# CVPR23/Depth-guided-Texture-Diffusion-for-Image-Semantic-Segmentation

Hardware: NVIDIA B200
Metric: rgbd_images_per_sec_384 (higher is better)
Workload: dtype bf16

## Files before the change

### depth-guided-texture-diffusion-for-image-semantic-segmentation_b200/csrc/common.cuh

```cuda
#pragma once
#include <cuda_bf16.h>
#include <cuda_runtime.h>
#include <stdint.h>
#include <stdio.h>

#include "../../include/dgtd_ops.h"

#if defined(__CUDA_ARCH__) && (__CUDA_ARCH__ < 1000)
#error "libdgtd_ops targets sm_100a only"
#endif

namespace dgtd {

void set_error(const char* fmt, ...);
void count_launch(int n = 1);

#define DGTD_CHECK_ARG(cond, ...)        \
  do {                                   \
    if (!(cond)) {                       \
      ::dgtd::set_error(__VA_ARGS__);    \
      return -1;                         \
    }                                    \
  } while (0)

#define DGTD_LAUNCH_CHECK(name)                                                  \
  do {                                                                           \
    cudaError_t e__ = cudaGetLastError();                                        \
    if (e__ != cudaSuccess) {                                                    \
      ::dgtd::set_error("%s: launch failed: %s", name, cudaGetErrorString(e__)); \
      return -2;                                                                 \
    }                                                                            \
    ::dgtd::count_launch();                                                      \
  } while (0)

static inline int cdiv(int64_t a, int64_t b) { return (int)((a + b - 1) / b); }

__device__ __forceinline__ float warp_sum(float v) {
#pragma unroll
  for (int o = 16; o > 0; o >>= 1) v += __shfl_xor_sync(0xffffffffu, v, o);
  return v;
}

__device__ __forceinline__ float gelu_erf(float x) {
  return 0.5f * x * (1.0f + erff(x * 0.70710678118654752440f));
}

__device__ __forceinline__ float sigmoidf_acc(float x) { return 1.0f / (1.0f + expf(-x)); }

template <int ACT>
__device__ __forceinline__ float apply_act(float x) {
  if (ACT == DGTD_ACT_GELU) return gelu_erf(x);
  if (ACT == DGTD_ACT_RELU) return fmaxf(x, 0.0f);
  return x;
}

__device__ __forceinline__ float to_float(float v) { return v; }
__device__ __forceinline__ float to_float(__nv_bfloat16 v) { return __bfloat162float(v); }

template <typename T>
__device__ __forceinline__ T from_float(float v);
template <>
__device__ __forceinline__ float from_float<float>(float v) { return v; }
template <>
__device__ __forceinline__ __nv_bfloat16 from_float<__nv_bfloat16>(float v) {
  return __float2bfloat16_rn(v);
}

__device__ __forceinline__ void store1(float* p, float v) { *p = v; }
__device__ __forceinline__ void store1(__nv_bfloat16* p, float v) { *p = __float2bfloat16_rn(v); }
__device__ __forceinline__ void store4(float* p, float a, float b, float c, float d) {
  *reinterpret_cast<float4*>(p) = make_float4(a, b, c, d);
}
__device__ __forceinline__ void store4(__nv_bfloat16* p, float a, float b, float c, float d) {
  __nv_bfloat162 lo = __floats2bfloat162_rn(a, b), hi = __floats2bfloat162_rn(c, d);
  uint2 u;
  u.x = *reinterpret_cast<uint32_t*>(&lo);
  u.y = *reinterpret_cast<uint32_t*>(&hi);
  *reinterpret_cast<uint2*>(p) = u;
}
__device__ __forceinline__ float4 load4(const float* p) {
  return *reinterpret_cast<const float4*>(p);
}
__device__ __forceinline__ float4 load4(const __nv_bfloat16* p) {
  uint2 u = *reinterpret_cast<const uint2*>(p);
  __nv_bfloat162 lo = *reinterpret_cast<__nv_bfloat162*>(&u.x);
  __nv_bfloat162 hi = *reinterpret_cast<__nv_bfloat162*>(&u.y);
  float2 a = __bfloat1622float2(lo), b = __bfloat1622float2(hi);
  return make_float4(a.x, a.y, b.x, b.y);
}

__device__ __forceinline__ uint64_t pk2(float a, float b) {
  uint64_t r;
  asm("mov.b64 %0, {%1, %2};" : "=l"(r) : "f"(a), "f"(b));
  return r;
}
__device__ __forceinline__ void up2(uint64_t r, float& a, float& b) {
  asm("mov.b64 {%0, %1}, %2;" : "=f"(a), "=f"(b) : "l"(r));
}
__device__ __forceinline__ uint64_t fma2(uint64_t a, uint64_t b, uint64_t c) {
  uint64_t d;
  asm("fma.rn.f32x2 %0, %1, %2, %3;" : "=l"(d) : "l"(a), "l"(b), "l"(c));
  return d;
}
__device__ __forceinline__ uint64_t mul2(uint64_t a, uint64_t b) {
  uint64_t d;
  asm("mul.rn.f32x2 %0, %1, %2;" : "=l"(d) : "l"(a), "l"(b));
  return d;
}
__device__ __forceinline__ uint64_t add2(uint64_t a, uint64_t b) {
  uint64_t d;
  asm("add.rn.f32x2 %0, %1, %2;" : "=l"(d) : "l"(a), "l"(b));
  return d;
}
__device__ __forceinline__ void bilinear_src(int dst, float scale, int in_size, int& i0, int& i1,
                                             float& l1) {
  float s = (dst + 0.5f) * scale - 0.5f;
  s = s < 0.f ? 0.f : s;
  i0 = (int)s;
  if (i0 > in_size - 1) i0 = in_size - 1;
  i1 = i0 + (i0 < in_size - 1 ? 1 : 0);
  l1 = s - (float)i0;
}

}
```

### depth-guided-texture-diffusion-for-image-semantic-segmentation_b200/csrc/dwconv_tma.cu

```cuda
#include "blackwell.cuh"
#include "common.cuh"

namespace dgtd {

int sm_count();
static inline int sm_count_dw() { return sm_count(); }

template <int SY, int SX, bool ADD, typename OT = float>
__global__ void __launch_bounds__(SY * SX * 32, 2)
dwconv7_tma_kernel(const __grid_constant__ CUtensorMap tmX, const float* __restrict__ wT,
                   const float* __restrict__ bias, const float* __restrict__ add, OT* __restrict__ y, int h,
                   int w, int C, int tiles_x, int tiles_y) {
  constexpr int TH = 4 * SY, TW = 8 * SX, PH = TH + 6, PW = TW + 6, NCH = 4;
  constexpr int TILE_FLOATS = PH * PW * 32;
  constexpr uint32_t TILE_BYTES = TILE_FLOATS * 4;
  extern __shared__ __align__(128) float xs[];
  __shared__ uint64_t bar[2];

  int bid = blockIdx.x;
  const int cgs = C >> 7;
  const int cg = bid % cgs; bid /= cgs;
  const int tx = bid % tiles_x; bid /= tiles_x;
  const int ty = bid % tiles_y;
  const int b = bid / tiles_y;
  const int warp = threadIdx.x >> 5, lane = threadIdx.x & 31;
  const int sy = warp / SX, sx = warp - sy * SX;
  const int x0 = tx * TW, y0 = ty * TH;

  if (threadIdx.x == 0) {
    bw::prefetch_tmap(&tmX);
    bw::mbar_init(&bar[0], 1);
    bw::mbar_init(&bar[1], 1);
    bw::fence_mbar_init();
  }
  __syncthreads();
  if (threadIdx.x == 0) {
    bw::mbar_arrive_expect_tx(&bar[0], TILE_BYTES);
    bw::tma_load_4d(&tmX, &bar[0], xs, cg * 128, x0 - 3, y0 - 3, b);
  }

#pragma unroll 1
  for (int i = 0; i < NCH; ++i) {
    const int c = cg * 128 + i * 32 + lane;
    if (threadIdx.x == 0 && i + 1 < NCH) {
      bw::fence_proxy_async_smem();
      bw::mbar_arrive_expect_tx(&bar[(i + 1) & 1], TILE_BYTES);
      bw::tma_load_4d(&tmX, &bar[(i + 1) & 1], xs + ((i + 1) & 1) * TILE_FLOATS, cg * 128 + (i + 1) * 32, x0 - 3,
                      y0 - 3, b);
    }
    uint64_t w2[49];
#pragma unroll
    for (int k = 0; k < 49; ++k) {
      const float t = __ldg(wT + (int64_t)k * C + c);
      w2[k] = pk2(t, t);
    }
    const float bc = bias ? __ldg(bias + c) : 0.f;
    uint64_t acc[2][8];
#pragma unroll
    for (int q = 0; q < 2; ++q)
#pragma unroll
      for (int j = 0; j < 8; ++j) acc[q][j] = pk2(bc, bc);

    bw::mbar_wait(&bar[i & 1], (i >> 1) & 1);
    const float* base = xs + (i & 1) * TILE_FLOATS + ((4 * sy) * PW + 8 * sx) * 32 + lane;
#pragma unroll
    for (int iy = 0; iy < 9; ++iy) {
      uint64_t pr[14];
#pragma unroll
      for (int j = 0; j < 14; ++j) {
        const volatile float* p0 = base + (iy * PW + j) * 32;
        pr[j] = pk2(p0[0], p0[PW * 32]);
      }
#pragma unroll
      for (int q = 0; q < 2; ++q) {
        const int ky = iy - 2 * q;
        if (ky < 0 || ky >= 7) continue;
#pragma unroll
        for (int kx = 0; kx < 7; ++kx)
#pragma unroll
          for (int j = 0; j < 8; ++j) acc[q][j] = fma2(w2[ky * 7 + kx], pr[j + kx], acc[q][j]);
      }
    }
    if (ADD) {
      float av[4][8];
#pragma unroll
      for (int a = 0; a < 4; ++a)
#pragma unroll
        for (int j = 0; j < 8; ++j) {
          const int oy = y0 + 4 * sy + a, ox = x0 + 8 * sx + j;
          av[a][j] = (oy < h && ox < w) ? __ldg(add + (((int64_t)b * h + oy) * w + ox) * C + c) : 0.f;
        }
#pragma unroll
      for (int q = 0; q < 2; ++q)
#pragma unroll
        for (int j = 0; j < 8; ++j) acc[q][j] = add2(acc[q][j], pk2(av[2 * q][j], av[2 * q + 1][j]));
    }
    {
      const int oy0 = y0 + 4 * sy, ox0 = x0 + 8 * sx;
      OT* yp = y + (((int64_t)b * h + oy0) * w + ox0) * C + c;
      const int rs = w * C;
      if (oy0 + 4 <= h && ox0 + 8 <= w) {
#pragma unroll
        for (int q = 0; q < 2; ++q)
#pragma unroll
          for (int j = 0; j < 8; ++j) {
            float v0, v1;
            up2(acc[q][j], v0, v1);
            store1(yp + (2 * q) * rs + j * C, v0);
            store1(yp + (2 * q + 1) * rs + j * C, v1);
          }
      } else {
#pragma unroll
        for (int q = 0; q < 2; ++q)
#pragma unroll
          for (int j = 0; j < 8; ++j) {
            float v0, v1;
            up2(acc[q][j], v0, v1);
            if (ox0 + j < w) {
              if (oy0 + 2 * q < h) store1(yp + (2 * q) * rs + j * C, v0);
              if (oy0 + 2 * q + 1 < h) store1(yp + (2 * q + 1) * rs + j * C, v1);
            }
          }
      }
    }
    __syncthreads();
  }
}


template <int SY, int SX, bool ADD, typename OT>
__global__ void __launch_bounds__(SY * SX * 32, 2)
dwconv7_tma_persist_kernel(const __grid_constant__ CUtensorMap tmX, const __grid_constant__ CUtensorMap tmW,
                           const float* __restrict__ bias, const float* __restrict__ add, OT* __restrict__ y, int h,
                           int w, int C, int tiles_x, int tiles_y, int num_items) {
  constexpr int TH = 4 * SY, TW = 8 * SX, PH = TH + 6, PW = TW + 6;
  constexpr int TILE_FLOATS = PH * PW * 32;
  constexpr uint32_t TILE_BYTES = TILE_FLOATS * 4, W_BYTES = 49 * 32 * 4;
  extern __shared__ __align__(128) float xs[];
  float* wbuf = xs + 2 * TILE_FLOATS;
  __shared__ uint64_t bar[3];

  const int warp = threadIdx.x >> 5, lane = threadIdx.x & 31;
  const int sy = warp / SX, sx = warp - sy * SX;
  const int nch = C >> 5;
  auto issue_tile = [&](int item, int buf) {
    const int chunk = item % nch;
    int t = item / nch;
    const int tx = t % tiles_x; t /= tiles_x;
    const int ty = t % tiles_y;
    const int b = t / tiles_y;
    bw::mbar_arrive_expect_tx(&bar[buf], TILE_BYTES);
    bw::tma_load_4d(&tmX, &bar[buf], xs + buf * TILE_FLOATS, chunk * 32, tx * TW - 3, ty * TH - 3, b);
  };
  auto issue_weights = [&](int item) {
    bw::mbar_arrive_expect_tx(&bar[2], W_BYTES);
    bw::tma_load_2d(&tmW, &bar[2], wbuf, (item % nch) * 32, 0);
  };
  if (threadIdx.x == 0) {
    bw::prefetch_tmap(&tmX);
    bw::prefetch_tmap(&tmW);
    bw::mbar_init(&bar[0], 1);
    bw::mbar_init(&bar[1], 1);
    bw::mbar_init(&bar[2], 1);
    bw::fence_mbar_init();
  }
  __syncthreads();
  if (threadIdx.x == 0 && (int)blockIdx.x < num_items) {
    issue_tile(blockIdx.x, 0);
    issue_weights(blockIdx.x);
  }
  int it = 0;
#pragma unroll 1
  for (int item = blockIdx.x; item < num_items; item += gridDim.x, ++it) {
    const int next = item + gridDim.x;
    if (threadIdx.x == 0 && next < num_items) {
      bw::fence_proxy_async_smem();
      issue_tile(next, (it + 1) & 1);
    }
    const int chunk = item % nch;
    int t = item / nch;
    const int tx = t % tiles_x; t /= tiles_x;
    const int ty = t % tiles_y;
    const int b = t / tiles_y;
    const int x0 = tx * TW, y0 = ty * TH;
    const int c = chunk * 32 + lane;
    bw::mbar_wait(&bar[2], it & 1);
    uint64_t w2[49];
#pragma unroll
    for (int k = 0; k < 49; ++k) {
      const float tv = wbuf[k * 32 + lane];
      w2[k] = pk2(tv, tv);
    }
    __syncthreads();
    if (threadIdx.x == 0 && next < num_items) {
      bw::fence_proxy_async_smem();
      issue_weights(next);
    }
    const float bc = bias ? __ldg(bias + c) : 0.f;
    uint64_t acc[2][8];
#pragma unroll
    for (int q = 0; q < 2; ++q)
#pragma unroll
      for (int j = 0; j < 8; ++j) acc[q][j] = pk2(bc, bc);

    bw::mbar_wait(&bar[it & 1], (it >> 1) & 1);
    const float* base = xs + (it & 1) * TILE_FLOATS + ((4 * sy) * PW + 8 * sx) * 32 + lane;
#pragma unroll
    for (int iy = 0; iy < 9; ++iy) {
      uint64_t pr[14];
#pragma unroll
      for (int j = 0; j < 14; ++j) {
        const volatile float* p0 = base + (iy * PW + j) * 32;
        pr[j] = pk2(p0[0], p0[PW * 32]);
      }
#pragma unroll
      for (int q = 0; q < 2; ++q) {
        const int ky = iy - 2 * q;
        if (ky < 0 || ky >= 7) continue;
#pragma unroll
        for (int kx = 0; kx < 7; ++kx)
#pragma unroll
          for (int j = 0; j < 8; ++j) acc[q][j] = fma2(w2[ky * 7 + kx], pr[j + kx], acc[q][j]);
      }
    }
    if (ADD) {
      float av[4][8];
#pragma unroll
      for (int a = 0; a < 4; ++a)
#pragma unroll
        for (int j = 0; j < 8; ++j) {
          const int oy = y0 + 4 * sy + a, ox = x0 + 8 * sx + j;
          av[a][j] = (oy < h && ox < w) ? __ldg(add + (((int64_t)b * h + oy) * w + ox) * C + c) : 0.f;
        }
#pragma unroll
      for (int q = 0; q < 2; ++q)
#pragma unroll
        for (int j = 0; j < 8; ++j) acc[q][j] = add2(acc[q][j], pk2(av[2 * q][j], av[2 * q + 1][j]));
    }
    {
      const int oy0 = y0 + 4 * sy, ox0 = x0 + 8 * sx;
      OT* yp = y + (((int64_t)b * h + oy0) * w + ox0) * C + c;
      const int rs = w * C;
      if (oy0 + 4 <= h && ox0 + 8 <= w) {
#pragma unroll
        for (int q = 0; q < 2; ++q)
#pragma unroll
          for (int j = 0; j < 8; ++j) {
            float v0, v1;
            up2(acc[q][j], v0, v1);
            store1(yp + (2 * q) * rs + j * C, v0);
            store1(yp + (2 * q + 1) * rs + j * C, v1);
          }
      } else {
#pragma unroll
        for (int q = 0; q < 2; ++q)
#pragma unroll
          for (int j = 0; j < 8; ++j) {
            float v0, v1;
            up2(acc[q][j], v0, v1);
            if (ox0 + j < w) {
              if (oy0 + 2 * q < h) store1(yp + (2 * q) * rs + j * C, v0);
              if (oy0 + 2 * q + 1 < h) store1(yp + (2 * q + 1) * rs + j * C, v1);
            }
          }
      }
    }
    __syncthreads();
  }
}

template <int SY, int SX>
__global__ void __launch_bounds__(SY * SX * 32, 2)
dwconv7_wgrad_tma_kernel(const __grid_constant__ CUtensorMap tmX, const float* __restrict__ dy,
                         float* __restrict__ part, int h, int w, int C, int tiles_x, int tiles_y, int ntiles) {
  constexpr int TH = 4 * SY, TW = 8 * SX, PH = TH + 6, PW = TW + 6, NW = SY * SX;
  constexpr int TILE_FLOATS = PH * PW * 32;
  constexpr uint32_t TILE_BYTES = TILE_FLOATS * 4;
  static_assert(NW * 50 * 32 <= 2 * TILE_FLOATS, "reduction scratch must fit in the tile buffers");
  extern __shared__ __align__(128) float xs[];
  __shared__ uint64_t bar[2];

  const int chunk = blockIdx.x, P = gridDim.y;
  const int warp = threadIdx.x >> 5, lane = threadIdx.x & 31;
  const int sy = warp / SX, sx = warp - sy * SX;
  const int c = chunk * 32 + lane;

  auto issue = [&](int t, int buf) {
    const int tx = t % tiles_x;
    const int r = t / tiles_x;
    const int ty = r % tiles_y, b = r / tiles_y;
    bw::mbar_arrive_expect_tx(&bar[buf], TILE_BYTES);
    bw::tma_load_4d(&tmX, &bar[buf], xs + buf * TILE_FLOATS, chunk * 32, tx * TW - 3, ty * TH - 3, b);
  };
  if (threadIdx.x == 0) {
    bw::prefetch_tmap(&tmX);
    bw::mbar_init(&bar[0], 1);
    bw::mbar_init(&bar[1], 1);
    bw::fence_mbar_init();
  }
  __syncthreads();
  if (threadIdx.x == 0) issue(blockIdx.y, 0);

  float acc[50];
#pragma unroll
  for (int k = 0; k < 50; ++k) acc[k] = 0.f;

  int it = 0;
#pragma unroll 1
  for (int t = blockIdx.y; t < ntiles; t += P, ++it) {
    if (threadIdx.x == 0 && t + P < ntiles) {
      bw::fence_proxy_async_smem();
      issue(t + P, (it + 1) & 1);
    }
    const int tx = t % tiles_x;
    const int r = t / tiles_x;
    const int ty = r % tiles_y, b = r / tiles_y;
    const int oy0 = ty * TH + 4 * sy, ox0 = tx * TW + 8 * sx;
    float g[4][8];
#pragma unroll
    for (int a = 0; a < 4; ++a)
#pragma unroll
      for (int j = 0; j < 8; ++j) {
        const int oy = oy0 + a, ox = ox0 + j;
        g[a][j] = (oy < h && ox < w) ? __ldg(dy + (((int64_t)b * h + oy) * w + ox) * C + c) : 0.f;
        acc[49] += g[a][j];
      }
    bw::mbar_wait(&bar[it & 1], (it >> 1) & 1);
    const float* base = xs + (it & 1) * TILE_FLOATS + ((4 * sy) * PW + 8 * sx) * 32 + lane;
#pragma unroll
    for (int iy = 0; iy < 10; ++iy) {
      float in[14];
#pragma unroll
      for (int j = 0; j < 14; ++j) in[j] = base[(iy * PW + j) * 32];
#pragma unroll
      for (int a = 0; a < 4; ++a) {
        const int ky = iy - a;
        if (ky < 0 || ky >= 7) continue;
#pragma unroll
        for (int kx = 0; kx < 7; ++kx)
#pragma unroll
          for (int j = 0; j < 8; ++j) acc[ky * 7 + kx] = fmaf(g[a][j], in[j + kx], acc[ky * 7 + kx]);
      }
    }
    __syncthreads();
  }
  float* red = xs;
#pragma unroll
  for (int k = 0; k < 50; ++k) red[(warp * 50 + k) * 32 + lane] = acc[k];
  __syncthreads();
  for (int i = threadIdx.x; i < 50 * 32; i += NW * 32) {
    float v = 0.f;
#pragma unroll
    for (int q = 0; q < NW; ++q) v += red[q * 50 * 32 + i];
    part[((int64_t)blockIdx.y * 50 + (i >> 5)) * C + chunk * 32 + (i & 31)] = v;
  }
}

template <typename OT, int VPL>
__global__ void __launch_bounds__(256)
ln_rows_kernel(const float* __restrict__ y, const float* __restrict__ ln_w, const float* __restrict__ ln_b,
               OT* __restrict__ out, int64_t rows, int C, float eps) {
  const int64_t row = (int64_t)blockIdx.x * 8 + (threadIdx.x >> 5);
  if (row >= rows) return;
  const int lane = threadIdx.x & 31;
  const float* p = y + row * C;
  float4 v[VPL];
  float s = 0.f;
#pragma unroll
  for (int j = 0; j < VPL; ++j) {
    v[j] = *reinterpret_cast<const float4*>(p + (j * 32 + lane) * 4);
    s += (v[j].x + v[j].y) + (v[j].z + v[j].w);
  }
  const float mean = warp_sum(s) / C;
  float q = 0.f;
#pragma unroll
  for (int j = 0; j < VPL; ++j) {
    float a = v[j].x - mean, b = v[j].y - mean, c = v[j].z - mean, d = v[j].w - mean;
    q += (a * a + b * b) + (c * c + d * d);
  }
  const float rstd = 1.0f / sqrtf(warp_sum(q) / C + eps);
  OT* o = out + row * C;
#pragma unroll
  for (int j = 0; j < VPL; ++j) {
    const int c0 = (j * 32 + lane) * 4;
    float4 g = *reinterpret_cast<const float4*>(ln_w + c0), be = *reinterpret_cast<const float4*>(ln_b + c0);
    store4(o + c0, (v[j].x - mean) * rstd * g.x + be.x, (v[j].y - mean) * rstd * g.y + be.y,
           (v[j].z - mean) * rstd * g.z + be.z, (v[j].w - mean) * rstd * g.w + be.w);
  }
}

template <int LPR, int V, int U>
__global__ void __launch_bounds__(256)
row_stats_bf16_kernel(const __nv_bfloat16* __restrict__ y, float2* __restrict__ stats, int64_t rows, int C, float eps) {
  constexpr int RPP = 32 / LPR;
  constexpr int RPW = RPP * U;
  const int lane = threadIdx.x & 31, sub = lane / LPR, l = lane % LPR;
  const int64_t row0 = ((int64_t)blockIdx.x * 8 + (threadIdx.x >> 5)) * RPW + sub;
  uint4 raw[U][V];
#pragma unroll
  for (int u = 0; u < U; ++u) {
    const int64_t row = row0 + u * RPP;
#pragma unroll
    for (int j = 0; j < V; ++j) {
      raw[u][j] = make_uint4(0u, 0u, 0u, 0u);
      if (row < rows) raw[u][j] = __ldg(reinterpret_cast<const uint4*>(y + row * C + (j * LPR + l) * 8));
    }
  }
  const float inv_c = 1.0f / C;
#pragma unroll
  for (int u = 0; u < U; ++u) {
    float f[V][8];
    float s = 0.f;
#pragma unroll
    for (int j = 0; j < V; ++j) {
      const uint32_t w4[4] = {raw[u][j].x, raw[u][j].y, raw[u][j].z, raw[u][j].w};
#pragma unroll
      for (int e = 0; e < 4; ++e) {
        f[j][2 * e] = __uint_as_float(w4[e] << 16);
        f[j][2 * e + 1] = __uint_as_float(w4[e] & 0xffff0000u);
      }
      s += ((f[j][0] + f[j][1]) + (f[j][2] + f[j][3])) + ((f[j][4] + f[j][5]) + (f[j][6] + f[j][7]));
    }
#pragma unroll
    for (int o = LPR / 2; o > 0; o >>= 1) s += __shfl_xor_sync(0xffffffffu, s, o);
    const float mean = s * inv_c;
    float q = 0.f;
#pragma unroll
    for (int j = 0; j < V; ++j) {
#pragma unroll
      for (int e = 0; e < 8; e += 2) {
        const float a = f[j][e] - mean, b = f[j][e + 1] - mean;
        q += a * a + b * b;
      }
    }
#pragma unroll
    for (int o = LPR / 2; o > 0; o >>= 1) q += __shfl_xor_sync(0xffffffffu, q, o);
    const int64_t row = row0 + u * RPP;
    if (l == 0 && row < rows) stats[row] = make_float2(mean, 1.0f / sqrtf(q * inv_c + eps));
  }
}

static int row_stats_grid(int64_t rows, int rows_per_block) { return (int)cdiv(rows, rows_per_block); }

int row_stats_bf16(const __nv_bfloat16* y, float2* stats, int64_t rows, int C, float eps, cudaStream_t s) {
  if (reinterpret_cast<uintptr_t>(y) & 15) {
    set_error("row_stats: the matrix must be 16-byte aligned");
    return -1;
  }
  switch (C / 128) {
    case 1: row_stats_bf16_kernel<16, 1, 4><<<row_stats_grid(rows, 64), 256, 0, s>>>(y, stats, rows, C, eps); break;
    case 2: row_stats_bf16_kernel<32, 1, 4><<<row_stats_grid(rows, 32), 256, 0, s>>>(y, stats, rows, C, eps); break;
    case 4: row_stats_bf16_kernel<32, 2, 2><<<row_stats_grid(rows, 16), 256, 0, s>>>(y, stats, rows, C, eps); break;
    case 8: row_stats_bf16_kernel<32, 4, 1><<<row_stats_grid(rows, 8), 256, 0, s>>>(y, stats, rows, C, eps); break;
    default:
      set_error("row_stats: C=%d must be 128*{1,2,4,8}", C);
      return -1;
  }
  return 0;
}

template <int SY, int SX, bool ADD, typename OT>
static int dw_launch_persist(const CUtensorMap& tm, const float* wT, const float* bias, const float* add, OT* y, int B, int h,
                             int w, int C, cudaStream_t s) {
  constexpr int PH = 4 * SY + 6, PW = 8 * SX + 6;
  constexpr int SMEM = 2 * PH * PW * 128 + 49 * 32 * 4 + 128;
  auto kern = dwconv7_tma_persist_kernel<SY, SX, ADD, OT>;
  static bool configured = false;
  if (!configured) {
    cudaError_t e = cudaFuncSetAttribute(kern, cudaFuncAttributeMaxDynamicSharedMemorySize, SMEM);
    if (e != cudaSuccess) {
      set_error("dwconv7_tma(persistent): cannot opt in to %d B smem: %s", SMEM, cudaGetErrorString(e));
      return -2;
    }
    configured = true;
  }
  CUtensorMap tmW;
  {
    const uint64_t dims[2] = {(uint64_t)C, 49}, strides[1] = {(uint64_t)C * 4};
    const uint32_t box[2] = {32, 49};
    int rc = make_tmap(&tmW, wT, CU_TENSOR_MAP_DATA_TYPE_FLOAT32, 2, dims, strides, box, CU_TENSOR_MAP_SWIZZLE_NONE);
    if (rc) return rc;
  }
  const int tiles_x = cdiv(w, 8 * SX), tiles_y = cdiv(h, 4 * SY);
  const int64_t items = (int64_t)B * tiles_x * tiles_y * (C / 32);
  if (items > 0x7fffffff) {
    set_error("dwconv7_tma(persistent): too many items");
    return -1;
  }
  const int slots = 2 * sm_count_dw();
  const int grid = items < slots ? (int)items : slots;
  kern<<<grid, SY * SX * 32, SMEM, s>>>(tm, tmW, bias, add, y, h, w, C, tiles_x, tiles_y, (int)items);
  return 0;
}

template <int SY, int SX>
static int dw_launch_bf16(const CUtensorMap& tm, const float* wT, const float* bias, __nv_bfloat16* y, int B, int h, int w,
                          int C, cudaStream_t s) {
  if ((reinterpret_cast<uintptr_t>(wT) & 15) == 0)
    return dw_launch_persist<SY, SX, false, __nv_bfloat16>(tm, wT, bias, nullptr, y, B, h, w, C, s);
  constexpr int PH = 4 * SY + 6, PW = 8 * SX + 6;
  constexpr int SMEM = 2 * PH * PW * 128 + 128;
  auto kern = dwconv7_tma_kernel<SY, SX, false, __nv_bfloat16>;
  static bool configured = false;
  if (!configured) {
    cudaError_t e = cudaFuncSetAttribute(kern, cudaFuncAttributeMaxDynamicSharedMemorySize, SMEM);
    if (e != cudaSuccess) {
      set_error("dwconv7_tma(bf16): cannot opt in to %d B smem: %s", SMEM, cudaGetErrorString(e));
      return -2;
    }
    configured = true;
  }
  const int tiles_x = cdiv(w, 8 * SX), tiles_y = cdiv(h, 4 * SY);
  const int64_t blocks = (int64_t)B * tiles_x * tiles_y * (C / 128);
  kern<<<(unsigned)blocks, SY * SX * 32, SMEM, s>>>(tm, wT, bias, nullptr, y, h, w, C, tiles_x, tiles_y);
  return 0;
}

template <int SY, int SX>
static int dw_launch(const CUtensorMap& tm, const float* wT, const float* bias, const float* add, float* y, int B,
                     int h, int w, int C, cudaStream_t s) {
  if ((reinterpret_cast<uintptr_t>(wT) & 15) == 0) {
    if (add) return dw_launch_persist<SY, SX, true, float>(tm, wT, bias, add, y, B, h, w, C, s);
    return dw_launch_persist<SY, SX, false, float>(tm, wT, bias, nullptr, y, B, h, w, C, s);
  }
  constexpr int PH = 4 * SY + 6, PW = 8 * SX + 6;
  constexpr int SMEM = 2 * PH * PW * 128 + 128;
  static bool configured = false;
  if (!configured) {
    cudaError_t e = cudaFuncSetAttribute(dwconv7_tma_kernel<SY, SX, false>, cudaFuncAttributeMaxDynamicSharedMemorySize, SMEM);
    if (e == cudaSuccess)
      e = cudaFuncSetAttribute(dwconv7_tma_kernel<SY, SX, true>, cudaFuncAttributeMaxDynamicSharedMemorySize, SMEM);
    if (e != cudaSuccess) {
      set_error("dwconv7_tma: cannot opt in to %d B smem: %s", SMEM, cudaGetErrorString(e));
      return -2;
    }
    configured = true;
  }
  const int tiles_x = cdiv(w, 8 * SX), tiles_y = cdiv(h, 4 * SY);
  const int64_t blocks = (int64_t)B * tiles_x * tiles_y * (C / 128);
  if (add)
    dwconv7_tma_kernel<SY, SX, true><<<(unsigned)blocks, SY * SX * 32, SMEM, s>>>(tm, wT, bias, add, y, h, w, C, tiles_x, tiles_y);
  else
    dwconv7_tma_kernel<SY, SX, false><<<(unsigned)blocks, SY * SX * 32, SMEM, s>>>(tm, wT, bias, add, y, h, w, C, tiles_x, tiles_y);
  return 0;
}

template <typename OT>
static int ln_rows_launch(const float* y, const float* ln_w, const float* ln_b, OT* out, int64_t rows, int C,
                          float eps, cudaStream_t s) {
  const int blocks = cdiv(rows, 8);
  switch (C / 128) {
    case 1: ln_rows_kernel<OT, 1><<<blocks, 256, 0, s>>>(y, ln_w, ln_b, out, rows, C, eps); break;
    case 2: ln_rows_kernel<OT, 2><<<blocks, 256, 0, s>>>(y, ln_w, ln_b, out, rows, C, eps); break;
    case 4: ln_rows_kernel<OT, 4><<<blocks, 256, 0, s>>>(y, ln_w, ln_b, out, rows, C, eps); break;
    case 8: ln_rows_kernel<OT, 8><<<blocks, 256, 0, s>>>(y, ln_w, ln_b, out, rows, C, eps); break;
    default:
      set_error("dwconv7_ln(tma): C=%d must be 128*{1,2,4,8}", C);
      return -1;
  }
  return 0;
}

int dwconv7_tma(const float* x, const float* wT, const float* dw_b, const float* add, float* y, int B, int h, int w,
                int C, cudaStream_t s) {
  if (C % 128 || C > 1024 || (reinterpret_cast<uintptr_t>(x) & 15)) return 1;
  const int SX = (w % 24 == 0 && w % 16 != 0) ? 3 : 2;
  const int SY = (h % 8 == 0 || h > 12) ? 2 : 3;
  CUtensorMap tm;
  {
    PFN_tmapEncodeTiled enc = get_tmap_encoder();
    if (!enc) return -3;
    cuuint64_t gd[4] = {(cuuint64_t)C, (cuuint64_t)w, (cuuint64_t)h, (cuuint64_t)B};
    cuuint64_t gs[3] = {(cuuint64_t)C * 4, (cuuint64_t)w * C * 4, (cuuint64_t)h * w * C * 4};
    cuuint32_t bx[4] = {32, (cuuint32_t)(8 * SX + 6), (cuuint32_t)(4 * SY + 6), 1};
    cuuint32_t es[4] = {1, 1, 1, 1};
    CUresult r = enc(&tm, CU_TENSOR_MAP_DATA_TYPE_FLOAT32, 4, const_cast<float*>(x), gd, gs, bx, es,
                     CU_TENSOR_MAP_INTERLEAVE_NONE, CU_TENSOR_MAP_SWIZZLE_NONE, CU_TENSOR_MAP_L2_PROMOTION_L2_128B,
                     CU_TENSOR_MAP_FLOAT_OOB_FILL_NONE);
    if (r != CUDA_SUCCESS) {
      set_error("dwconv7(tma): cuTensorMapEncodeTiled failed (%d) for x (%d,%d,%d,%d)", (int)r, B, h, w, C);
      return -3;
    }
  }
  int rc;
  if (SY == 2 && SX == 2) rc = dw_launch<2, 2>(tm, wT, dw_b, add, y, B, h, w, C, s);
  else if (SY == 2 && SX == 3) rc = dw_launch<2, 3>(tm, wT, dw_b, add, y, B, h, w, C, s);
  else if (SY == 3 && SX == 2) rc = dw_launch<3, 2>(tm, wT, dw_b, add, y, B, h, w, C, s);
  else rc = dw_launch<3, 3>(tm, wT, dw_b, add, y, B, h, w, C, s);
  if (rc) return rc;
  cudaError_t e = cudaGetLastError();
  if (e != cudaSuccess) {
    set_error("dwconv7_tma: launch failed: %s", cudaGetErrorString(e));
    return -2;
  }
  count_launch();
  return 0;
}


template <int SY, int SX>
static int dwg_launch(const CUtensorMap& tm, const float* dy, float* part, int P, int B, int h, int w, int C,
                      cudaStream_t s) {
  constexpr int PH = 4 * SY + 6, PW = 8 * SX + 6;
  constexpr int SMEM = 2 * PH * PW * 128 + 128;
  auto kern = dwconv7_wgrad_tma_kernel<SY, SX>;
  static bool configured = false;
  if (!configured) {
    cudaError_t e = cudaFuncSetAttribute(kern, cudaFuncAttributeMaxDynamicSharedMemorySize, SMEM);
    if (e != cudaSuccess) {
      set_error("dwconv7_wgrad_tma: cannot opt in to %d B smem: %s", SMEM, cudaGetErrorString(e));
      return -2;
    }
    configured = true;
  }
  const int tiles_x = cdiv(w, 8 * SX), tiles_y = cdiv(h, 4 * SY);
  kern<<<dim3(C / 32, P), SY * SX * 32, SMEM, s>>>(tm, dy, part, h, w, C, tiles_x, tiles_y, B * tiles_x * tiles_y);
  return 0;
}

static int dw_tile_shape(int h, int w, int* SY, int* SX) {
  *SX = (w % 24 == 0 && w % 16 != 0) ? 3 : 2;
  *SY = (h % 8 == 0 || h > 12) ? 2 : 3;
  return 0;
}

static int dw_make_tmap(CUtensorMap* tm, const float* x, int B, int h, int w, int C, int SY, int SX) {
  PFN_tmapEncodeTiled enc = get_tmap_encoder();
  if (!enc) return -3;
  cuuint64_t gd[4] = {(cuuint64_t)C, (cuuint64_t)w, (cuuint64_t)h, (cuuint64_t)B};
  cuuint64_t gs[3] = {(cuuint64_t)C * 4, (cuuint64_t)w * C * 4, (cuuint64_t)h * w * C * 4};
  cuuint32_t bx[4] = {32, (cuuint32_t)(8 * SX + 6), (cuuint32_t)(4 * SY + 6), 1};
  cuuint32_t es[4] = {1, 1, 1, 1};
  CUresult r = enc(tm, CU_TENSOR_MAP_DATA_TYPE_FLOAT32, 4, const_cast<float*>(x), gd, gs, bx, es,
                   CU_TENSOR_MAP_INTERLEAVE_NONE, CU_TENSOR_MAP_SWIZZLE_NONE, CU_TENSOR_MAP_L2_PROMOTION_L2_128B,
                   CU_TENSOR_MAP_FLOAT_OOB_FILL_NONE);
  if (r != CUDA_SUCCESS) {
    set_error("dwconv7(tma): cuTensorMapEncodeTiled failed (%d) for x (%d,%d,%d,%d)", (int)r, B, h, w, C);
    return -3;
  }
  return 0;
}

int dwconv7_wgrad_tma(const float* x, const float* dy, float* part, int max_parts, int* parts, int B, int h, int w,
                      int C, cudaStream_t s) {
  if (C % 128 || (reinterpret_cast<uintptr_t>(x) & 15) || (int64_t)B * h * w < 2048) return 1;
  int SY, SX;
  dw_tile_shape(h, w, &SY, &SX);
  const int ntiles = B * cdiv(w, 8 * SX) * cdiv(h, 4 * SY);
  int P = cdiv(2 * 148, C / 32);
  if (P > ntiles) P = ntiles;
  if (P > max_parts) P = max_parts;
  if (P < 1) return 1;
  CUtensorMap tm;
  int rc = dw_make_tmap(&tm, x, B, h, w, C, SY, SX);
  if (rc) return rc;
  if (SY == 2 && SX == 2) rc = dwg_launch<2, 2>(tm, dy, part, P, B, h, w, C, s);
  else if (SY == 2 && SX == 3) rc = dwg_launch<2, 3>(tm, dy, part, P, B, h, w, C, s);
  else if (SY == 3 && SX == 2) rc = dwg_launch<3, 2>(tm, dy, part, P, B, h, w, C, s);
  else rc = dwg_launch<3, 3>(tm, dy, part, P, B, h, w, C, s);
  if (rc) return rc;
  cudaError_t e = cudaGetLastError();
  if (e != cudaSuccess) {
    set_error("dwconv7_wgrad_tma: launch failed: %s", cudaGetErrorString(e));
    return -2;
  }
  count_launch();
  *parts = P;
  return 0;
}

int dwconv7_stats_tma(const float* x, const float* wT, const float* dw_b, __nv_bfloat16* y, float2* stats, int B, int h,
                      int w, int C, float eps, cudaStream_t s) {
  if (C % 128 || C > 1024 || (reinterpret_cast<uintptr_t>(x) & 15)) return 1;
  int SY, SX;
  dw_tile_shape(h, w, &SY, &SX);
  CUtensorMap tm;
  int rc = dw_make_tmap(&tm, x, B, h, w, C, SY, SX);
  if (rc) return rc;
  if (SY == 2 && SX == 2) rc = dw_launch_bf16<2, 2>(tm, wT, dw_b, y, B, h, w, C, s);
  else if (SY == 2 && SX == 3) rc = dw_launch_bf16<2, 3>(tm, wT, dw_b, y, B, h, w, C, s);
  else if (SY == 3 && SX == 2) rc = dw_launch_bf16<3, 2>(tm, wT, dw_b, y, B, h, w, C, s);
  else rc = dw_launch_bf16<3, 3>(tm, wT, dw_b, y, B, h, w, C, s);
  if (rc) return rc;
  cudaError_t e = cudaGetLastError();
  if (e != cudaSuccess) {
    set_error("dwconv7_stats_tma: launch failed: %s", cudaGetErrorString(e));
    return -2;
  }
  count_launch();
  rc = row_stats_bf16(y, stats, (int64_t)B * h * w, C, eps, s);
  if (rc) return rc;
  e = cudaGetLastError();
  if (e != cudaSuccess) {
    set_error("row_stats: launch failed: %s", cudaGetErrorString(e));
    return -2;
  }
  count_launch();
  return 0;
}

int dwconv7_ln_tma(const float* x, const float* wT, const float* dw_b, const float* ln_w, const float* ln_b,
                   float* ws, void* out, int out_dtype, int B, int h, int w, int C, float eps, cudaStream_t s) {
  int rc = dwconv7_tma(x, wT, dw_b, nullptr, ws, B, h, w, C, s);
  if (rc) return rc;
  const int64_t rows = (int64_t)B * h * w;
  return out_dtype == DGTD_BF16 ? ln_rows_launch(ws, ln_w, ln_b, (__nv_bfloat16*)out, rows, C, eps, s)
                                : ln_rows_launch(ws, ln_w, ln_b, (float*)out, rows, C, eps, s);
}

int ln_rows_any(const float* y, const float* ln_w, const float* ln_b, void* out, int out_dtype, int64_t rows, int C,
                float eps, cudaStream_t s) {
  return out_dtype == DGTD_BF16 ? ln_rows_launch(y, ln_w, ln_b, (__nv_bfloat16*)out, rows, C, eps, s)
                                : ln_rows_launch(y, ln_w, ln_b, (float*)out, rows, C, eps, s);
}

}
```

Baseline: 5347.

## Pin channel chunk per persistent CTA and pack channel pairs in dwconv7

```diff
diff --git a/depth-guided-texture-diffusion-for-image-semantic-segmentation_b200/csrc/common.cuh b/depth-guided-texture-diffusion-for-image-semantic-segmentation_b200/csrc/common.cuh
--- a/depth-guided-texture-diffusion-for-image-semantic-segmentation_b200/csrc/common.cuh
+++ b/depth-guided-texture-diffusion-for-image-semantic-segmentation_b200/csrc/common.cuh
@@ -68,6 +68,10 @@
 
 __device__ __forceinline__ void store1(float* p, float v) { *p = v; }
 __device__ __forceinline__ void store1(__nv_bfloat16* p, float v) { *p = __float2bfloat16_rn(v); }
+__device__ __forceinline__ void store2(float* p, float a, float b) { *reinterpret_cast<float2*>(p) = make_float2(a, b); }
+__device__ __forceinline__ void store2(__nv_bfloat16* p, float a, float b) {
+  *reinterpret_cast<__nv_bfloat162*>(p) = __floats2bfloat162_rn(a, b);
+}
 __device__ __forceinline__ void store4(float* p, float a, float b, float c, float d) {
   *reinterpret_cast<float4*>(p) = make_float4(a, b, c, d);
 }
diff --git a/depth-guided-texture-diffusion-for-image-semantic-segmentation_b200/csrc/dwconv_tma.cu b/depth-guided-texture-diffusion-for-image-semantic-segmentation_b200/csrc/dwconv_tma.cu
--- a/depth-guided-texture-diffusion-for-image-semantic-segmentation_b200/csrc/dwconv_tma.cu
+++ b/depth-guided-texture-diffusion-for-image-semantic-segmentation_b200/csrc/dwconv_tma.cu
@@ -6,145 +6,27 @@
 int sm_count();
 static inline int sm_count_dw() { return sm_count(); }
 
-template <int SY, int SX, bool ADD, typename OT = float>
-__global__ void __launch_bounds__(SY * SX * 32, 2)
-dwconv7_tma_kernel(const __grid_constant__ CUtensorMap tmX, const float* __restrict__ wT,
-                   const float* __restrict__ bias, const float* __restrict__ add, OT* __restrict__ y, int h,
-                   int w, int C, int tiles_x, int tiles_y) {
-  constexpr int TH = 4 * SY, TW = 8 * SX, PH = TH + 6, PW = TW + 6, NCH = 4;
+template <int SY, int SX>
+constexpr int dw_ctas_per_sm() { return 2 * 2 * (4 * SY + 6) * (8 * SX + 6) * 128 <= 227 * 1024 ? 2 : 1; }
+
+template <int SY, int SX, bool ADD, typename OT>
+__global__ void __launch_bounds__(SY * SX * 32, dw_ctas_per_sm<SY, SX>())
+dwconv7_tma_persist_kernel(const __grid_constant__ CUtensorMap tmX, const float* __restrict__ wT,
+                           const float* __restrict__ bias, const float* __restrict__ add, OT* __restrict__ y, int h,
+                           int w, int C, int tiles_x, int tiles_y, int num_items) {
+  constexpr int TH = 4 * SY, TW = 8 * SX, PH = TH + 6, PW = TW + 6;
   constexpr int TILE_FLOATS = PH * PW * 32;
   constexpr uint32_t TILE_BYTES = TILE_FLOATS * 4;
   extern __shared__ __align__(128) float xs[];
   __shared__ uint64_t bar[2];
 
-  int bid = blockIdx.x;
-  const int cgs = C >> 7;
-  const int cg = bid % cgs; bid /= cgs;
-  const int tx = bid % tiles_x; bid /= tiles_x;
-  const int ty = bid % tiles_y;
-  const int b = bid / tiles_y;
   const int warp = threadIdx.x >> 5, lane = threadIdx.x & 31;
   const int sy = warp / SX, sx = warp - sy * SX;
-  const int x0 = tx * TW, y0 = ty * TH;
-
-  if (threadIdx.x == 0) {
-    bw::prefetch_tmap(&tmX);
-    bw::mbar_init(&bar[0], 1);
-    bw::mbar_init(&bar[1], 1);
-    bw::fence_mbar_init();
-  }
-  __syncthreads();
-  if (threadIdx.x == 0) {
-    bw::mbar_arrive_expect_tx(&bar[0], TILE_BYTES);
-    bw::tma_load_4d(&tmX, &bar[0], xs, cg * 128, x0 - 3, y0 - 3, b);
-  }
-
-#pragma unroll 1
-  for (int i = 0; i < NCH; ++i) {
-    const int c = cg * 128 + i * 32 + lane;
-    if (threadIdx.x == 0 && i + 1 < NCH) {
-      bw::fence_proxy_async_smem();
-      bw::mbar_arrive_expect_tx(&bar[(i + 1) & 1], TILE_BYTES);
-      bw::tma_load_4d(&tmX, &bar[(i + 1) & 1], xs + ((i + 1) & 1) * TILE_FLOATS, cg * 128 + (i + 1) * 32, x0 - 3,
-                      y0 - 3, b);
-    }
-    uint64_t w2[49];
-#pragma unroll
-    for (int k = 0; k < 49; ++k) {
-      const float t = __ldg(wT + (int64_t)k * C + c);
-      w2[k] = pk2(t, t);
-    }
-    const float bc = bias ? __ldg(bias + c) : 0.f;
-    uint64_t acc[2][8];
-#pragma unroll
-    for (int q = 0; q < 2; ++q)
-#pragma unroll
-      for (int j = 0; j < 8; ++j) acc[q][j] = pk2(bc, bc);
-
-    bw::mbar_wait(&bar[i & 1], (i >> 1) & 1);
-    const float* base = xs + (i & 1) * TILE_FLOATS + ((4 * sy) * PW + 8 * sx) * 32 + lane;
-#pragma unroll
-    for (int iy = 0; iy < 9; ++iy) {
-      uint64_t pr[14];
-#pragma unroll
-      for (int j = 0; j < 14; ++j) {
-        const volatile float* p0 = base + (iy * PW + j) * 32;
-        pr[j] = pk2(p0[0], p0[PW * 32]);
-      }
-#pragma unroll
-      for (int q = 0; q < 2; ++q) {
-        const int ky = iy - 2 * q;
-        if (ky < 0 || ky >= 7) continue;
-#pragma unroll
-        for (int kx = 0; kx < 7; ++kx)
-#pragma unroll
-          for (int j = 0; j < 8; ++j) acc[q][j] = fma2(w2[ky * 7 + kx], pr[j + kx], acc[q][j]);
-      }
-    }
-    if (ADD) {
-      float av[4][8];
-#pragma unroll
-      for (int a = 0; a < 4; ++a)
-#pragma unroll
-        for (int j = 0; j < 8; ++j) {
-          const int oy = y0 + 4 * sy + a, ox = x0 + 8 * sx + j;
-          av[a][j] = (oy < h && ox < w) ? __ldg(add + (((int64_t)b * h + oy) * w + ox) * C + c) : 0.f;
-        }
-#pragma unroll
-      for (int q = 0; q < 2; ++q)
-#pragma unroll
-        for (int j = 0; j < 8; ++j) acc[q][j] = add2(acc[q][j], pk2(av[2 * q][j], av[2 * q + 1][j]));
-    }
-    {
-      const int oy0 = y0 + 4 * sy, ox0 = x0 + 8 * sx;
-      OT* yp = y + (((int64_t)b * h + oy0) * w + ox0) * C + c;
-      const int rs = w * C;
-      if (oy0 + 4 <= h && ox0 + 8 <= w) {
-#pragma unroll
-        for (int q = 0; q < 2; ++q)
-#pragma unroll
-          for (int j = 0; j < 8; ++j) {
-            float v0, v1;
-            up2(acc[q][j], v0, v1);
-            store1(yp + (2 * q) * rs + j * C, v0);
-            store1(yp + (2 * q + 1) * rs + j * C, v1);
-          }
-      } else {
-#pragma unroll
-        for (int q = 0; q < 2; ++q)
-#pragma unroll
-          for (int j = 0; j < 8; ++j) {
-            float v0, v1;
-            up2(acc[q][j], v0, v1);
-            if (ox0 + j < w) {
-              if (oy0 + 2 * q < h) store1(yp + (2 * q) * rs + j * C, v0);
-              if (oy0 + 2 * q + 1 < h) store1(yp + (2 * q + 1) * rs + j * C, v1);
-            }
-          }
-      }
-    }
-    __syncthreads();
-  }
-}
-
-
-template <int SY, int SX, bool ADD, typename OT>
-__global__ void __launch_bounds__(SY * SX * 32, 2)
-dwconv7_tma_persist_kernel(const __grid_constant__ CUtensorMap tmX, const __grid_constant__ CUtensorMap tmW,
-                           const float* __restrict__ bias, const float* __restrict__ add, OT* __restrict__ y, int h,
-                           int w, int C, int tiles_x, int tiles_y, int num_items) {
-  constexpr int TH = 4 * SY, TW = 8 * SX, PH = TH + 6, PW = TW + 6;
-  constexpr int TILE_FLOATS = PH * PW * 32;
-  constexpr uint32_t TILE_BYTES = TILE_FLOATS * 4, W_BYTES = 49 * 32 * 4;
-  extern __shared__ __align__(128) float xs[];
-  float* wbuf = xs + 2 * TILE_FLOATS;
-  __shared__ uint64_t bar[3];
-
-  const int warp = threadIdx.x >> 5, lane = threadIdx.x & 31;
-  const int sy = warp / SX, sx = warp - sy * SX;
+  const int half = lane >> 4;
   const int nch = C >> 5;
+  const int chunk = blockIdx.x % nch;
+  const int c = chunk * 32 + 2 * (lane & 15);
   auto issue_tile = [&](int item, int buf) {
-    const int chunk = item % nch;
     int t = item / nch;
     const int tx = t % tiles_x; t /= tiles_x;
     const int ty = t % tiles_y;
@@ -152,23 +34,19 @@
     bw::mbar_arrive_expect_tx(&bar[buf], TILE_BYTES);
     bw::tma_load_4d(&tmX, &bar[buf], xs + buf * TILE_FLOATS, chunk * 32, tx * TW - 3, ty * TH - 3, b);
   };
-  auto issue_weights = [&](int item) {
-    bw::mbar_arrive_expect_tx(&bar[2], W_BYTES);
-    bw::tma_load_2d(&tmW, &bar[2], wbuf, (item % nch) * 32, 0);
-  };
   if (threadIdx.x == 0) {
     bw::prefetch_tmap(&tmX);
-    bw::prefetch_tmap(&tmW);
     bw::mbar_init(&bar[0], 1);
     bw::mbar_init(&bar[1], 1);
-    bw::mbar_init(&bar[2], 1);
     bw::fence_mbar_init();
   }
   __syncthreads();
-  if (threadIdx.x == 0 && (int)blockIdx.x < num_items) {
-    issue_tile(blockIdx.x, 0);
-    issue_weights(blockIdx.x);
-  }
+  if (threadIdx.x == 0 && (int)blockIdx.x < num_items) issue_tile(blockIdx.x, 0);
+  uint64_t w2[49];
+#pragma unroll
+  for (int k = 0; k < 49; ++k) w2[k] = pk2(__ldg(wT + (int64_t)k * C + c), __ldg(wT + (int64_t)k * C + c + 1));
+  const uint64_t b2 = bias ? pk2(__ldg(bias + c), __ldg(bias + c + 1)) : pk2(0.f, 0.f);
+
   int it = 0;
 #pragma unroll 1
   for (int item = blockIdx.x; item < num_items; item += gridDim.x, ++it) {
@@ -177,93 +55,73 @@
       bw::fence_proxy_async_smem();
       issue_tile(next, (it + 1) & 1);
     }
-    const int chunk = item % nch;
     int t = item / nch;
     const int tx = t % tiles_x; t /= tiles_x;
     const int ty = t % tiles_y;
     const int b = t / tiles_y;
-    const int x0 = tx * TW, y0 = ty * TH;
-    const int c = chunk * 32 + lane;
-    bw::mbar_wait(&bar[2], it & 1);
-    uint64_t w2[49];
-#pragma unroll
-    for (int k = 0; k < 49; ++k) {
-      const float tv = wbuf[k * 32 + lane];
-      w2[k] = pk2(tv, tv);
-    }
-    __syncthreads();
-    if (threadIdx.x == 0 && next < num_items) {
-      bw::fence_proxy_async_smem();
-      issue_weights(next);
-    }
-    const float bc = bias ? __ldg(bias + c) : 0.f;
-    uint64_t acc[2][8];
-#pragma unroll
-    for (int q = 0; q < 2; ++q)
-#pragma unroll
-      for (int j = 0; j < 8; ++j) acc[q][j] = pk2(bc, bc);
+    uint64_t acc[4][4];
+#pragma unroll
+    for (int a = 0; a < 4; ++a)
+#pragma unroll
+      for (int j = 0; j < 4; ++j) acc[a][j] = b2;
 
     bw::mbar_wait(&bar[it & 1], (it >> 1) & 1);
-    const float* base = xs + (it & 1) * TILE_FLOATS + ((4 * sy) * PW + 8 * sx) * 32 + lane;
-#pragma unroll
-    for (int iy = 0; iy < 9; ++iy) {
-      uint64_t pr[14];
-#pragma unroll
-      for (int j = 0; j < 14; ++j) {
-        const volatile float* p0 = base + (iy * PW + j) * 32;
-        pr[j] = pk2(p0[0], p0[PW * 32]);
+    const float* base = xs + (it & 1) * TILE_FLOATS + ((4 * sy) * PW + 8 * sx + 4 * half) * 32 + 2 * (lane & 15);
+#pragma unroll
+    for (int iy = 0; iy < 10; ++iy) {
+      uint64_t in[10];
+#pragma unroll
+      for (int j = 0; j < 10; ++j) in[j] = *reinterpret_cast<const uint64_t*>(base + (iy * PW + j) * 32);
+#pragma unroll
+      for (int a = 0; a < 4; ++a) {
+        const int ky = iy - a;
+        if (ky < 0 || ky >= 7) continue;
+#pragma unroll
+        for (int kx = 0; kx < 7; ++kx)
+#pragma unroll
+          for (int j = 0; j < 4; ++j) acc[a][j] = fma2(w2[ky * 7 + kx], in[j + kx], acc[a][j]);
       }
-#pragma unroll
-      for (int q = 0; q < 2; ++q) {
-        const int ky = iy - 2 * q;
-        if (ky < 0 || ky >= 7) continue;
-#pragma unroll
-        for (int kx = 0; kx < 7; ++kx)
-#pragma unroll
-          for (int j = 0; j < 8; ++j) acc[q][j] = fma2(w2[ky * 7 + kx], pr[j + kx], acc[q][j]);
+    }
+    const int oy0 = ty * TH + 4 * sy, ox0 = tx * TW + 8 * sx + 4 * half;
+    const bool interior = oy0 + 4 <= h && ox0 + 4 <= w;
+    const int64_t p0 = ((int64_t)b * h + oy0) * w + ox0;
+    if (ADD) {
+#pragma unroll
+      for (int a0 = 0; a0 < 4; a0 += 2) {
+        uint64_t av[2][4];
+#pragma unroll
+        for (int a = 0; a < 2; ++a)
+#pragma unroll
+          for (int j = 0; j < 4; ++j)
+            av[a][j] = (interior || (oy0 + a0 + a < h && ox0 + j < w))
+                           ? __ldg(reinterpret_cast<const unsigned long long*>(add + (p0 + (int64_t)(a0 + a) * w + j) * C + c))
+                           : 0ull;
+#pragma unroll
+        for (int a = 0; a < 2; ++a)
+#pragma unroll
+          for (int j = 0; j < 4; ++j) acc[a0 + a][j] = add2(acc[a0 + a][j], av[a][j]);
       }
     }
-    if (ADD) {
-      float av[4][8];
+    OT* yp = y + p0 * C + c;
+    const int rs = w * C;
+    if (interior) {
 #pragma unroll
       for (int a = 0; a < 4; ++a)
 #pragma unroll
-        for (int j = 0; j < 8; ++j) {
-          const int oy = y0 + 4 * sy + a, ox = x0 + 8 * sx + j;
-          av[a][j] = (oy < h && ox < w) ? __ldg(add + (((int64_t)b * h + oy) * w + ox) * C + c) : 0.f;
+        for (int j = 0; j < 4; ++j) {
+          float v0, v1;
+          up2(acc[a][j], v0, v1);
+          store2(yp + a * rs + j * C, v0, v1);
         }
-#pragma unroll
-      for (int q = 0; q < 2; ++q)
-#pragma unroll
-        for (int j = 0; j < 8; ++j) acc[q][j] = add2(acc[q][j], pk2(av[2 * q][j], av[2 * q + 1][j]));
-    }
-    {
-      const int oy0 = y0 + 4 * sy, ox0 = x0 + 8 * sx;
-      OT* yp = y + (((int64_t)b * h + oy0) * w + ox0) * C + c;
-      const int rs = w * C;
-      if (oy0 + 4 <= h && ox0 + 8 <= w) {
-#pragma unroll
-        for (int q = 0; q < 2; ++q)
-#pragma unroll
-          for (int j = 0; j < 8; ++j) {
-            float v0, v1;
-            up2(acc[q][j], v0, v1);
-            store1(yp + (2 * q) * rs + j * C, v0);
-            store1(yp + (2 * q + 1) * rs + j * C, v1);
-          }
-      } else {
-#pragma unroll
-        for (int q = 0; q < 2; ++q)
-#pragma unroll
-          for (int j = 0; j < 8; ++j) {
-            float v0, v1;
-            up2(acc[q][j], v0, v1);
-            if (ox0 + j < w) {
-              if (oy0 + 2 * q < h) store1(yp + (2 * q) * rs + j * C, v0);
-              if (oy0 + 2 * q + 1 < h) store1(yp + (2 * q + 1) * rs + j * C, v1);
-            }
-          }
-      }
+    } else {
+#pragma unroll
+      for (int a = 0; a < 4; ++a)
+#pragma unroll
+        for (int j = 0; j < 4; ++j) {
+          float v0, v1;
+          up2(acc[a][j], v0, v1);
+          if (oy0 + a < h && ox0 + j < w) store2(yp + a * rs + j * C, v0, v1);
+        }
     }
     __syncthreads();
   }
@@ -463,7 +321,7 @@
 static int dw_launch_persist(const CUtensorMap& tm, const float* wT, const float* bias, const float* add, OT* y, int B, int h,
                              int w, int C, cudaStream_t s) {
   constexpr int PH = 4 * SY + 6, PW = 8 * SX + 6;
-  constexpr int SMEM = 2 * PH * PW * 128 + 49 * 32 * 4 + 128;
+  constexpr int SMEM = 2 * PH * PW * 128 + 128;
   auto kern = dwconv7_tma_persist_kernel<SY, SX, ADD, OT>;
   static bool configured = false;
   if (!configured) {
@@ -474,75 +332,25 @@
     }
     configured = true;
   }
-  CUtensorMap tmW;
-  {
-    const uint64_t dims[2] = {(uint64_t)C, 49}, strides[1] = {(uint64_t)C * 4};
-    const uint32_t box[2] = {32, 49};
-    int rc = make_tmap(&tmW, wT, CU_TENSOR_MAP_DATA_TYPE_FLOAT32, 2, dims, strides, box, CU_TENSOR_MAP_SWIZZLE_NONE);
-    if (rc) return rc;
-  }
   const int tiles_x = cdiv(w, 8 * SX), tiles_y = cdiv(h, 4 * SY);
-  const int64_t items = (int64_t)B * tiles_x * tiles_y * (C / 32);
+  const int nch = C / 32;
+  const int64_t items = (int64_t)B * tiles_x * tiles_y * nch;
   if (items > 0x7fffffff) {
     set_error("dwconv7_tma(persistent): too many items");
     return -1;
   }
-  const int slots = 2 * sm_count_dw();
-  const int grid = items < slots ? (int)items : slots;
-  kern<<<grid, SY * SX * 32, SMEM, s>>>(tm, tmW, bias, add, y, h, w, C, tiles_x, tiles_y, (int)items);
-  return 0;
-}
-
-template <int SY, int SX>
-static int dw_launch_bf16(const CUtensorMap& tm, const float* wT, const float* bias, __nv_bfloat16* y, int B, int h, int w,
-                          int C, cudaStream_t s) {
-  if ((reinterpret_cast<uintptr_t>(wT) & 15) == 0)
-    return dw_launch_persist<SY, SX, false, __nv_bfloat16>(tm, wT, bias, nullptr, y, B, h, w, C, s);
-  constexpr int PH = 4 * SY + 6, PW = 8 * SX + 6;
-  constexpr int SMEM = 2 * PH * PW * 128 + 128;
-  auto kern = dwconv7_tma_kernel<SY, SX, false, __nv_bfloat16>;
-  static bool configured = false;
-  if (!configured) {
-    cudaError_t e = cudaFuncSetAttribute(kern, cudaFuncAttributeMaxDynamicSharedMemorySize, SMEM);
-    if (e != cudaSuccess) {
-      set_error("dwconv7_tma(bf16): cannot opt in to %d B smem: %s", SMEM, cudaGetErrorString(e));
-      return -2;
-    }
-    configured = true;
-  }
-  const int tiles_x = cdiv(w, 8 * SX), tiles_y = cdiv(h, 4 * SY);
-  const int64_t blocks = (int64_t)B * tiles_x * tiles_y * (C / 128);
-  kern<<<(unsigned)blocks, SY * SX * 32, SMEM, s>>>(tm, wT, bias, nullptr, y, h, w, C, tiles_x, tiles_y);
+  int grid = dw_ctas_per_sm<SY, SX>() * sm_count_dw() / nch * nch;
+  if (grid < nch) grid = nch;
+  if (items < grid) grid = (int)items;
+  kern<<<grid, SY * SX * 32, SMEM, s>>>(tm, wT, bias, add, y, h, w, C, tiles_x, tiles_y, (int)items);
   return 0;
 }
 
 template <int SY, int SX>
 static int dw_launch(const CUtensorMap& tm, const float* wT, const float* bias, const float* add, float* y, int B,
                      int h, int w, int C, cudaStream_t s) {
-  if ((reinterpret_cast<uintptr_t>(wT) & 15) == 0) {
-    if (add) return dw_launch_persist<SY, SX, true, float>(tm, wT, bias, add, y, B, h, w, C, s);
-    return dw_launch_persist<SY, SX, false, float>(tm, wT, bias, nullptr, y, B, h, w, C, s);
-  }
-  constexpr int PH = 4 * SY + 6, PW = 8 * SX + 6;
-  constexpr int SMEM = 2 * PH * PW * 128 + 128;
-  static bool configured = false;
-  if (!configured) {
-    cudaError_t e = cudaFuncSetAttribute(dwconv7_tma_kernel<SY, SX, false>, cudaFuncAttributeMaxDynamicSharedMemorySize, SMEM);
-    if (e == cudaSuccess)
-      e = cudaFuncSetAttribute(dwconv7_tma_kernel<SY, SX, true>, cudaFuncAttributeMaxDynamicSharedMemorySize, SMEM);
-    if (e != cudaSuccess) {
-      set_error("dwconv7_tma: cannot opt in to %d B smem: %s", SMEM, cudaGetErrorString(e));
-      return -2;
-    }
-    configured = true;
-  }
-  const int tiles_x = cdiv(w, 8 * SX), tiles_y = cdiv(h, 4 * SY);
-  const int64_t blocks = (int64_t)B * tiles_x * tiles_y * (C / 128);
-  if (add)
-    dwconv7_tma_kernel<SY, SX, true><<<(unsigned)blocks, SY * SX * 32, SMEM, s>>>(tm, wT, bias, add, y, h, w, C, tiles_x, tiles_y);
-  else
-    dwconv7_tma_kernel<SY, SX, false><<<(unsigned)blocks, SY * SX * 32, SMEM, s>>>(tm, wT, bias, add, y, h, w, C, tiles_x, tiles_y);
-  return 0;
+  if (add) return dw_launch_persist<SY, SX, true, float>(tm, wT, bias, add, y, B, h, w, C, s);
+  return dw_launch_persist<SY, SX, false, float>(tm, wT, bias, nullptr, y, B, h, w, C, s);
 }
 
 template <typename OT>
@@ -563,7 +371,8 @@
 
 int dwconv7_tma(const float* x, const float* wT, const float* dw_b, const float* add, float* y, int B, int h, int w,
                 int C, cudaStream_t s) {
-  if (C % 128 || C > 1024 || (reinterpret_cast<uintptr_t>(x) & 15)) return 1;
+  if (C % 128 || C > 1024 || (reinterpret_cast<uintptr_t>(x) & 15) || ((reinterpret_cast<uintptr_t>(y) | reinterpret_cast<uintptr_t>(add)) & 7))
+    return 1;
   const int SX = (w % 24 == 0 && w % 16 != 0) ? 3 : 2;
   const int SY = (h % 8 == 0 || h > 12) ? 2 : 3;
   CUtensorMap tm;
@@ -671,16 +480,16 @@
 
 int dwconv7_stats_tma(const float* x, const float* wT, const float* dw_b, __nv_bfloat16* y, float2* stats, int B, int h,
                       int w, int C, float eps, cudaStream_t s) {
-  if (C % 128 || C > 1024 || (reinterpret_cast<uintptr_t>(x) & 15)) return 1;
+  if (C % 128 || C > 1024 || (reinterpret_cast<uintptr_t>(x) & 15) || (reinterpret_cast<uintptr_t>(y) & 3)) return 1;
   int SY, SX;
   dw_tile_shape(h, w, &SY, &SX);
   CUtensorMap tm;
   int rc = dw_make_tmap(&tm, x, B, h, w, C, SY, SX);
   if (rc) return rc;
-  if (SY == 2 && SX == 2) rc = dw_launch_bf16<2, 2>(tm, wT, dw_b, y, B, h, w, C, s);
-  else if (SY == 2 && SX == 3) rc = dw_launch_bf16<2, 3>(tm, wT, dw_b, y, B, h, w, C, s);
-  else if (SY == 3 && SX == 2) rc = dw_launch_bf16<3, 2>(tm, wT, dw_b, y, B, h, w, C, s);
-  else rc = dw_launch_bf16<3, 3>(tm, wT, dw_b, y, B, h, w, C, s);
+  if (SY == 2 && SX == 2) rc = dw_launch_persist<2, 2, false, __nv_bfloat16>(tm, wT, dw_b, nullptr, y, B, h, w, C, s);
+  else if (SY == 2 && SX == 3) rc = dw_launch_persist<2, 3, false, __nv_bfloat16>(tm, wT, dw_b, nullptr, y, B, h, w, C, s);
+  else if (SY == 3 && SX == 2) rc = dw_launch_persist<3, 2, false, __nv_bfloat16>(tm, wT, dw_b, nullptr, y, B, h, w, C, s);
+  else rc = dw_launch_persist<3, 3, false, __nv_bfloat16>(tm, wT, dw_b, nullptr, y, B, h, w, C, s);
   if (rc) return rc;
   cudaError_t e = cudaGetLastError();
   if (e != cudaSuccess) {
```

New measurement: 5427, median of 6. +1.5%, better.
